# ishine/Prior-DiffuSE

Measured on AMD Instinct MI355X. Metric: enhanced-audio sec/sec (RTF), 6-step fast sampling, B=32, higher is better.
Workload: dtype f16x2; 1 GPU; B=32 x 4 s 16 kHz utterances per GPU, [B,2,401,161] spectrograms, GCRN prior + DiffUNet1 6-step sampling, STFT..ISTFT, seeded random weights; global_batch=32, frames=401, parallelism=batch-shard x1, graph=True, streams_per_gpu=1, batches_in_flight=3

## Files before the change

prior-diffuse_amd/csrc/gconv4.hip:

```cpp
#include <hip/hip_runtime.h>
#include <stdint.h>
#include <stdio.h>
#include <stdlib.h>

#include "pdse.h"
#include "pdse_internal.h"

#include "gconv_common.h"

#ifndef G4_CH
#define G4_CH 3
#endif

__device__ __forceinline__ float g4_load(const float* sbase, const unsigned byte_off) {
  float v;
  asm volatile("global_load_dword %0, %1, %2" : "=v"(v) : "v"(byte_off), "s"(sbase) : "memory");
  return v;
}
typedef float g4_f32x4 __attribute__((ext_vector_type(4)));
__device__ __forceinline__ g4_f32x4 g4_load16(const float* sbase, const unsigned byte_off) {
  g4_f32x4 v;
  asm volatile("global_load_dwordx4 %0, %1, %2" : "=v"(v) : "v"(byte_off), "s"(sbase) : "memory");
  return v;
}
// ... 308 lines not shown
    const int tap = kb / cbn, cb = kb - tap * cbn;
    int dt = 0, df = 0;
#pragma unroll
    for (int k = 0; k < 12; ++k) {
      dt = tap == k ? d.tap_dt[k] : dt;
      df = tap == k ? d.tap_df[k] : df;
    }
    const int tin = t + dt, fin = df;
    const bool inb = pvalid && fin >= 0 && fin < d.Fin && tin >= 0 && tin < d.Tin;
    const int64_t pos = inb ? (int64_t)b * d.in0.sb + (int64_t)tin * d.in0.st + (int64_t)fin * d.in0.sf : 0;
    float x[8];
    if constexpr (BLK) {
      const float* q = d.in0.ptr + pos + (int64_t)(2 * cb + h) * d.in0.sc;
      const float4 v0 = *reinterpret_cast<const float4*>(q), v1 = *reinterpret_cast<const float4*>(q + 4);
      x[0] = v0.x, x[1] = v0.y, x[2] = v0.z, x[3] = v0.w, x[4] = v1.x, x[5] = v1.y, x[6] = v1.z, x[7] = v1.w;
    } else {
      const float* q = d.in0.ptr + pos + (int64_t)(16 * cb + 8 * h) * d.in0.sc;
#pragma unroll
      for (int e = 0; e < 8; ++e) x[e] = q[(int64_t)e * d.in0.sc];
    }
#pragma unroll
    for (int e = 0; e < 8; ++e) x[e] = inb ? x[e] : 0.f;
    if (elu) {
#pragma unroll
      for (int e = 0; e < 8; ++e) x[e] = x[e] < 0.f ? fast_exp(x[e]) - 1.0f : x[e];
    }
    uint4 bp[NP];
    split_planes<NP>(x, bp, pow2i(PDSE_F16_ACT_EXP));
#pragma unroll
    for (int p = 0; p < NP; ++p) bimg[(kb * NP + p) * 64 + lane] = bp[p];
  }
  __syncthreads();

  const int mt0 = (blockIdx.y * 8 + wave) * MTW;
  if (mt0 >= mtiles) return;
  const uint4* const wl = reinterpret_cast<const uint4*>(d.w0) + lane;
  u32x4 a[MTW][NP];
  auto lda = [&](const int kb, const int m) {
    const u32x4* src = reinterpret_cast<const u32x4*>(wl + ((size_t)kb * mtiles + mt0 + m) * (NP * 64));
#pragma unroll
    for (int p = 0; p < NP; ++p) a[m][p] = src[p * 64];
  };
  f32x16 acc[MTW];
#pragma unroll
  for (int m = 0; m < MTW; ++m) {
#pragma unroll
    for (int r = 0; r < 16; ++r) acc[m][r] = 0.f;
    lda(0, m);
  }
  for (int kb = 0; kb < nkb; ++kb) {
    uint4 bp[NP];
#pragma unroll
    for (int p = 0; p < NP; ++p) bp[p] = bimg[(kb * NP + p) * 64 + lane];
    const int kn = min(kb + 1, nkb - 1);
#pragma unroll
    for (int m = 0; m < MTW; ++m) {
      acc[m] = g4_mma<NP>(a[m], bp, acc[m]);
      lda(kn, m);
    }
  }
  if constexpr (NP == 2) {
    const float us = pow2i(-(PDSE_F16_ACT_EXP + d.wexp));
#pragma unroll
    for (int m = 0; m < MTW; ++m)
#pragma unroll
      for (int r = 0; r < 16; ++r) acc[m][r] *= us;
  }
  gconv_epilogue_impl<PDSE_EPI_LINEAR, MTW, true>(d, tail_from_desc(d), acc, acc, b, t, 0, pvalid, lane, h, mt0, mtiles, 0);
}

template <bool BLK, int NP>
static int launch4f(const pdse_gconv_desc* d, hipStream_t s) {
  constexpr int MTW = 4;
  const int mtiles = (d->Cout + 31) / 32, nkb = d->ntaps * (d->in0.C >> 4);
  const long long N = (long long)d->B * d->Tout;
  const dim3 grid((unsigned)((N + 31) / 32), (mtiles + 8 * MTW - 1) / (8 * MTW)), block(512);
  const size_t lds = (size_t)nkb * NP * 64 * sizeof(uint4);
  static unsigned long long attr_mask = 0;
  if (lds > 64 * 1024 && pdse_lds_attr((const void*)gconv4_flat_kernel<MTW, BLK, NP>, &attr_mask, "gconv4 flat lds attribute")) return 1;
  hipLaunchKernelGGL((gconv4_flat_kernel<MTW, BLK, NP>), grid, block, lds, s, *d);
  return pdse_check_launch("gconv4 flat");
}

static int check4(const pdse_gconv_desc* d) {
  const bool two = d->in1.C > 0;
  const long long span0 = 4 * ((long long)d->B * d->in0.sb + 40ll * d->in0.sc), span1 = two ? 4 * ((long long)d->B * d->in1.sb + 40ll * d->in1.sc) : 0;
  auto blk_ok = [](const pdse_src& x) {
    return x.blk == 0 || (x.blk == 8 && !((x.sb | x.sc | x.st | x.sf) & 3) && (reinterpret_cast<uintptr_t>(x.ptr) & 15) == 0);
  };
  if (!blk_ok(d->in0) || (two && !blk_ok(d->in1)) || (two && d->in0.blk != d->in1.blk)) {
    pdse_set_error("gconv4: a channel-blocked source has blk = 8, strides in multiples of 4 floats and a 16-byte aligned base; "
                   "two sources are both blocked or both plain");
    return 1;
  }
  if (!(d->epi == PDSE_EPI_LINEAR || d->epi == PDSE_EPI_GLU) || (d->in0.C & 15) || (d->in1.C & 15) || d->in0.C == 0 || d->cin1 ||
      d->xf_mode != 0 || d->padrow != nullptr || d->ntaps > 12 || span0 >= (1ll << 32) || span1 >= (1ll << 32) ||
      (d->epi == PDSE_EPI_GLU && !d->w1) || (d->korder == 5 && (d->wexp < -40 || d->wexp > 40))) {
    pdse_set_error("gconv4: split-bf16 GEMM convolutions need LINEAR / GLU, channel counts in multiples of 16, <= 12 taps, "
                   "no load transform / pad row, 32-bit gather offsets");
    return 1;
  }
  if (d->flat && (d->flat != 1 || !(d->korder == 3 || d->korder == 5) || d->epi != PDSE_EPI_LINEAR || two || d->Fout != 1 ||
                  d->ntaps * (d->in0.C >> 4) > 32 || (d->Cout & 255) || d->out_cr != 1 || (long long)d->B * d->Tout > (1ll << 30))) {
    pdse_set_error("gconv4: the flat form takes korder 3 / 5 LINEAR launches of one source with Fout = 1, ntaps * C <= 512, "
                   "Cout in multiples of 256 and out_cr = 1");
    return 1;
  }
  return 0;
}

int pdse_gconv4_launch(const pdse_gconv_desc* d, hipStream_t s) {
  if (check4(d)) return 1;
  if (d->flat) {
    if (d->korder == 5) return d->in0.blk ? launch4f<true, 2>(d, s) : launch4f<false, 2>(d, s);
    return d->in0.blk ? launch4f<true, 3>(d, s) : launch4f<false, 3>(d, s);
  }
  const int mtiles = (d->Cout + 31) / 32;
  if (d->epi == PDSE_EPI_GLU) return mtiles >= 2 ? launch4<PDSE_EPI_GLU, 2>(d, s, mtiles) : launch4<PDSE_EPI_GLU, 1>(d, s, mtiles);
  if (mtiles >= 4) return launch4<PDSE_EPI_LINEAR, 4>(d, s, mtiles);
  if (mtiles >= 2) return launch4<PDSE_EPI_LINEAR, 2>(d, s, mtiles);
  return launch4<PDSE_EPI_LINEAR, 1>(d, s, mtiles);
}

template <int MT, bool BLK>
__global__ __launch_bounds__(512, 2) void gconv4_pair_kernel(const pdse_gconv_desc d, const pdse_gconv_desc e) {
  constexpr int NP = 2, FB = 64 * NP;
  constexpr int FR = 2 * MT, FR2 = 2 * FR;
  extern __shared__ uint4 ring[];
  const unsigned ring_base = (unsigned)(uintptr_t)ring;
  const int tid = threadIdx.x;
  const int lane = tid & 63, wave = tid >> 6;
  const int col = lane & 31, h = lane >> 5;
  const int b = blockIdx.y;
  const int P = d.Tout * d.Fout;
  const int p = (blockIdx.x * 8 + wave) * 32 + col;
  const bool pvalid = p < P;
  const int t = pvalid ? p / d.Fout : 0;
  const int j = pvalid ? p - t * d.Fout : 0;
  const int mtiles = (d.Cout + 31) >> 5;
  const int mt0 = blockIdx.z * MT;

  const int cbn0 = d.in0.C >> 4, cbn1 = d.in1.C >> 4;
  const int cps0 = (cbn0 + G4_CH - 1) / G4_CH, cps1 = (cbn1 + G4_CH - 1) / G4_CH;
  const int nch0 = d.ntaps * cps0, nch = nch0 + d.ntaps * cps1;

  auto uni = [](const int v) { return __builtin_amdgcn_readfirstlane(v); };
  auto decode = [&](const int ci) {
    g4_chunk c;
    c.s = uni(ci >= nch0);
    const int q = c.s ? ci - nch0 : ci, cps = c.s ? cps1 : cps0, cbn = c.s ? cbn1 : cbn0;
    c.tap = uni(q / cps);
    c.cb0 = uni((q - c.tap * cps) * G4_CH);
    c.n = uni(min(G4_CH, cbn - c.cb0));
    c.kb0 = uni((c.s ? d.ntaps * cbn0 : 0) + c.tap * cbn + c.cb0);
    return c;
  };
  auto dma = [&](const g4_chunk& c, const int buf) {
    const int nf = c.tap == 0 ? FR2 : FR;
    const int kb1 = (c.s ? cbn0 : 0) + c.cb0;
    const int npieces = c.n * nf * NP;
    for (int pc = __builtin_amdgcn_readfirstlane(wave); pc < npieces; pc += 8) {
      const int i = pc / (nf * NP), rem = pc - i * (nf * NP), f = rem / NP, part = rem - f * NP;
      const bool odd = f >= FR;
      const int g = odd ? f - FR : f, br = g / MT, m = g - br * MT;
      if (mt0 + m < mtiles) {
        const float* const w = odd ? (br ? e.w1 : e.w0) : (br ? d.w1 : d.w0);
        const uint4* src = reinterpret_cast<const uint4*>(w) + ((size_t)((odd ? kb1 : c.kb0) + i) * mtiles + mt0 + m) * FB + part * 64 + lane;
        glds16(src, ring + ((buf * G4_CH + i) * FR2 + f) * FB + part * 64);
      }
    }
  };
  auto gather = [&](const g4_chunk& c, g4_raw<BLK>& raw, bool& inb) {
    const bool s1 = c.s != 0;
    const float* const sptr = s1 ? d.in1.ptr : d.in0.ptr;
    const int64_t ssb = s1 ? d.in1.sb : d.in0.sb, ssc = s1 ? d.in1.sc : d.in0.sc, sst = s1 ? d.in1.st : d.in0.st,
                  ssf = s1 ? d.in1.sf : d.in0.sf;
    int dt = 0, df = 0;
#pragma unroll
    for (int k = 0; k < 12; ++k) {
      dt = c.tap == k ? d.tap_dt[k] : dt;
      df = c.tap == k ? d.tap_df[k] : df;
    }
    const int tin = t + dt, fin = j * d.sf_in + df;
    inb = pvalid && fin >= 0 && fin < d.Fin && tin >= 0 && tin < d.Tin;
    if constexpr (BLK) {
      const unsigned off = 4u * (unsigned)((inb ? (int64_t)b * ssb + (int64_t)tin * sst + (int64_t)fin * ssf : 0) + (int64_t)h * ssc);
#pragma unroll
      for (int i = 0; i < G4_CH; ++i) {
        if (i < c.n) {
          const float* base = sptr + (int64_t)(2 * (c.cb0 + i)) * ssc;
          raw.v[i][0] = g4_load16(base, off);
          raw.v[i][1] = g4_load16(base + 4, off);
        }
      }
    } else {
// ... 135 lines not shown
```

prior-diffuse_amd/nets.py:

```python
import ctypes as C

import numpy as np
import torch

from . import _lib as L
from . import packing as P

F0 = 161
BIG = 1 << 30

TAG_NONE, TAG_EPS_BLOCK, TAG_EPS_CONV1, TAG_TCM, TAG_PRIOR, TAG_LSTM, TAG_SIGNAL, TAG_EW = range(8)


class WeightBank:

    def __init__(self):
        self.items = {}
        self.keep = []
        self.owners = []

    def token(self, obj):
        if obj is None:
            return None
        for i, o in enumerate(self.owners):
# ... 132 lines not shown
            if hit is None:
                raise RuntimeError("range audit: the f16x2 operand at 0x%x lies in no buffer the builder named (PlanBase.named)" % addr)
            name, t = hit
            key = (name + suffix, kind)
            if key in seen:
                continue
            seen.add(key)
            out.append((name + suffix, t, kind, P.F16_ACT_EXP if kind == L.RANGE_F32 else 0,
                        None if box is None else dict(box, off=(addr - t.data_ptr()) // 2)))
        return out

    def finish(self):
        if self.plan is not None:
            self.plan.keep(self.ctx.keep, self.ctx.bank)

    def src(self, t, C_, sb, sc, st, sf, off=0, act=L.ACT_NONE, blk=0):
        return L.Src(Ctx.ptr(t, off), sb, sc, st, sf, C_, act, blk, 0)

    def gconv(self, *, in0, in1=None, Tin, Fin, taps, sf_in, W, Cout, bias0=None, bias0_sb=0,
              bias1=None, bias1_sb=0, epi=L.EPI_LINEAR, act=L.ACT_NONE, act_slope=0.0,
              padrow=None, padrow_sb=0, padrow_off=0, cin1=False, resid=None, out,
              out_strides, out_off=0, out_cr=1, B, Tout, Fout, tag=TAG_NONE, bias0_off=0, phase1=None, nx=None,
              bias1_off=0, bias_t0=None, label="gconv", s3=False, s3g=False, has_xf=False, flat=False):
        ctx = self.ctx
        d = L.GconvDesc()
        d.in0 = in0
        d.in1 = in1 if in1 is not None else L.Src(0, 0, 0, 0, 0, 0, 0)
        d.Tin, d.Fin = Tin, Fin
        d.padrow, d.padrow_sb = Ctx.ptr(padrow, padrow_off), padrow_sb
        ttaps = tuple((int(a), int(b)) for a, b in taps)
        tkey = ("taps", ttaps)
        tp = ctx.bank.items.get(tkey)
        if tp is None:
            ctx._banking += 1
            tp = ctx.bank.items[tkey] = self._up(P.taps_array(ttaps))
            ctx._banking -= 1
        d.taps, d.ntaps, d.sf_in = tp.data_ptr(), len(ttaps), sf_in
        for i, (dt_, df_) in enumerate(ttaps[:12]):
            d.tap_dt[i], d.tap_df[i] = dt_, df_
        d.cin1 = 1 if cin1 else 0
        c0, c1 = d.in0.C, d.in1.C
        pipelined_ok = padrow is None and not self.force_generic
        s3 = bool(s3) and pipelined_ok and epi == L.EPI_BIGLU and (
            ((c0, c1) == (32, 0) and len(ttaps) in (4, 6)) or ((c0, c1, len(ttaps)) == (2, 2, 10) and phase1 is None))
        s3g = (bool(s3g) and not s3 and pipelined_ok and epi in (L.EPI_LINEAR, L.EPI_GLU) and not cin1 and not has_xf
               and c0 > 0 and c0 % 16 == 0 and c1 % 16 == 0 and len(ttaps) <= 12)
        site = "%s:%d:%d:%d:%d:%d:%d:%d:%d" % (label, epi, len(ttaps), c0, c1, Cout, pipelined_ok, s3, s3g)
        if s3g:
            pack = lambda: P.gconv_gemm_fields(W(), len(ttaps), c0, c1, self.gemm_planes)
        elif s3:
            pack = lambda: P.gconv_s3_fields(W(), len(ttaps), c0 + c1)
        else:
            pack = lambda: P.gconv_fields(W(), len(ttaps), c0, c1, epi, cin1, pipelined_ok)
        self.apply(d, self.fields(site, pack))
        d.Cout = Cout
        if bias0 is not None:
            d.bias0 = Ctx.ptr(bias0, bias0_off)
        if bias1 is not None:
            d.bias1 = Ctx.ptr(bias1, bias1_off)
        d.bias0_sb, d.bias1_sb = bias0_sb, bias1_sb
        if bias_t0 is not None:
            d.bias0_t0, d.bias1_t0 = Ctx.ptr(bias_t0[0], bias_t0[1]), Ctx.ptr(bias_t0[0], bias_t0[2])
        d.epi, d.act, d.act_slope = epi, act, float(act_slope)
        if phase1 is not None and d.korder in (1, 2):
            d.p1mask, d.Fout1 = phase1["mask"], phase1["Fout1"]
        elif phase1 is not None and d.korder == 5 and epi == L.EPI_GLU:
            d.p1mask, d.Fout1 = phase1["mask"], phase1["Fout1"]
        if nx is not None:
            tiles = nx["tiles"]
            d.nx_n, d.nx_keep, d.nx_row0 = len(tiles), 1 if nx.get("keep") else 0, nx.get("row0", -1)
            for i, tl in enumerate(tiles):
                if tl.get("bias") is not None:
                    d.nx_bias[i] = Ctx.ptr(tl["bias"], tl.get("bias_off", 0))
                d.nx_bias_sb[i] = tl.get("bias_sb", 0)
                d.nx_out[i] = Ctx.ptr(tl["out"])
                d.nx_sb[i], d.nx_sc[i], d.nx_st[i], d.nx_sf[i] = tl["strides"]
                d.nx_off[i] = tl.get("off", 0)
                d.nx_add[i] = Ctx.ptr(tl.get("add"))
        d.resid = Ctx.ptr(resid)
        d.out = Ctx.ptr(out)
        d.out_sb, d.out_sc_hi, d.out_sc_lo, d.out_st, d.out_sf = out_strides
        d.out_off, d.out_cr = out_off, out_cr
        d.B, d.Tout, d.Fout = B, Tout, Fout
        d.flat = 1 if flat and s3g and d.korder in (3, 5) else 0
        self.add(d, tag)
        return d


def nchw(C_, T, F):
    return C_ * T * F, T * F, F, 1


def nchw_out(C_, T, F):
    return C_ * T * F, T * F, 0, F, 1


def nc8(C_, T, F):
    return C_ * T * F, T * F * 8, F * 8, 8


def nc8_out(C_, T, F):
    return C_ * T * F, T * F * 8, 1, F * 8, 8


class EpsNetPlan(PlanBase):

    ENC_F = [161, 79, 39, 19, 9, 4]
    fused_tcm = True
    chain_conv1 = True
    compose_stage1 = True
    split_bf16 = True
    split_tcm = True
    plane_h = True
    tcm_stack = True
    parity_planes = True
    planes = 2
    TCM_F16 = True
    NSLOT = 20

    def __init__(self, ctx, sd, B, T, time_cond=True, nsteps=1, plan=None, table=None, with_pre=None, split_bf16=None,
                 planes=None, plane_h=None, exclusive=False, frames=None):
        with_pre = time_cond if with_pre is None else with_pre
        if split_bf16 is not None:
            self.split_bf16 = bool(split_bf16)
        if planes is not None:
            if int(planes) not in (1, 2, 3):
                raise ValueError("planes is 3 (bf16x3), 2 (f16x2) or 1 (bf16 mode)")
            self.planes = int(planes)
        if plane_h is not None:
            self.plane_h = bool(plane_h)
        if self.planes == 1:
            self.plane_h = True
        self.tcm_planes = 3 if (self.planes == 2 and not self.TCM_F16) else self.planes
        self.use_tcm_stack = bool(self.tcm_stack and exclusive)
        self.frames = frames
        if frames is not None and (self.force_generic or not self.fused_tcm):
            raise ValueError("exact ragged batches need a fused TCM form (csrc/tcm.hip, csrc/tcm2.hip): the three-launch form has no frames table")
        self.sd = sd
        ok = (self.split_bf16 and self.chain_conv1 and self.compose_stage1 and time_cond and with_pre and not self.force_generic
              and all(float(P._np(sd[k])[0]) <= 1.0 for k in sd if k.endswith(".weight") and P._np(sd[k]).shape == (1,)))
        if not ok:
            if self.planes == 1:
                raise ValueError("bf16 mode needs the chained split-bf16 DiffUNet1 path (PReLU slopes <= 1)")
            self.plane_h = False
            if self.planes == 2:
                self.planes = self.tcm_planes = 3
        super().__init__(ctx, plan, ns=(ctx.bank.token(sd), bool(time_cond), bool(with_pre), self.fused_tcm, self.chain_conv1,
                                        self.compose_stage1, self.split_bf16, self.split_tcm,
                                        ctx.bank.token(table), str(self.plane_h), self.planes, self.parity_planes))
        self.sd, self.B, self.T, self.time_cond, self.nsteps = sd, B, T, time_cond, nsteps
        self.with_pre = with_pre
        a = ctx.alloc
        self.x = a(B, 2, T, F0)
        self.x_init = a(B, 2, T, F0) if self.with_pre else None
        self.out = a(B, 2, T, F0)
        self.H = a(B, 32, T + 1, F0)
        self.H2 = a(B, 32, T + 1, F0)
        self.Pskip = [[None] + [a(B + 1, 32, T, self.ENC_F[k]) for k in range(1, 5)] for _ in range(2)]
        self.zero32 = self.upw("zero32", lambda: np.zeros(32))
        self.en = [a(B, 64, T, f) for f in self.ENC_F[1:5]] + [a(B, 64, 4, T)]
        self.tcm_a, self.tcm_b = a(B, 256, T), a(B, 256, T)
        self.tcm_h, self.tcm_g = a(B, 64, T), a(B, 64, T)
        self.tcm_hs = [ctx.alloc_u16(*P.tcm2_hs_shape(B, T, self.tcm_planes)) for _ in range(2)]
        self._tcm_stack = None
        self.tcm_flags = torch.zeros(B * ((T + 31) // 32), dtype=torch.int32, device=ctx.device)
        self.tcm_status = torch.zeros(4, dtype=torch.int32, device=ctx.device)
        ctx.keep += [self.tcm_flags, self.tcm_status]
# ... 502 lines not shown
            if chained and k == 1 and self.compose_stage1:
                Fin = self._biconvglu_composed(step, src_x, src_i, o, ostr, nx)
            else:
                Fin = self._biconvglu(step, k, src_x, src_i, Fin, o, ostr, H=Hc, do_conv1=(k == 1 or not chained), nx=nx)
            if chained:
                Hc, Hn = Hn, Hc
            src_x, src_i = self.src(o, 64, *nchw(64, T, Fin)), None
        cur, nxt = self.en[4], self.tcm_a
        names = [("TCMs.%d.residual%d" % (i, j + 1), dil) for i in range(3) for j, dil in enumerate((1, 2, 4, 8, 16, 32))]
        if self.force_generic or not self.fused_tcm:
            for p, dil in names:
                self._residual(p, dil, cur, nxt)
                cur, nxt = nxt, (self.tcm_b if nxt is self.tcm_a else self.tcm_a)
        elif self.split_bf16 and self.split_tcm:
            hcur, hnxt = self.tcm_hs
            self._residual_split(None, 1, cur, None, None, hcur, names[0][0], mode=1)
            self._tcm_stack = [] if self.use_tcm_stack else None
            for n, (p, dil) in enumerate(names):
                p_next = names[n + 1][0] if n + 1 < len(names) else None
                self._residual_split(p, dil, cur, nxt, hcur, hnxt, p_next)
                cur, nxt = nxt, (self.tcm_b if nxt is self.tcm_a else self.tcm_a)
                hcur, hnxt = hnxt, hcur
            if self._tcm_stack:
                sd_ = L.Tcm2sDesc()
                for n, blk in enumerate(self._tcm_stack):
                    sd_.blk[n] = blk
                sd_.n = len(self._tcm_stack)
                sd_.flags, sd_.status = self.tcm_flags.data_ptr(), self.tcm_status.data_ptr()
                self.add(sd_, TAG_TCM)
            self._tcm_stack = None
        else:
            hcur, hnxt = self.tcm_h, self.tcm_g
            self._tcm_conv1(names[0][0], cur, hcur)
            for n, (p, dil) in enumerate(names):
                p_next = names[n + 1][0] if n + 1 < len(names) else None
                self._residual_fused(p, dil, cur, nxt, hcur, hnxt, p_next)
                cur, nxt = nxt, (self.tcm_b if nxt is self.tcm_a else self.tcm_a)
                hcur, hnxt = hnxt, hcur
        tcm_out = cur
        if self._plane_stage("dec"):
            self._decoders_planes(step, tcm_out, out)
            return out
        for di, de in enumerate(("de_real", "de_imag")):
            in0 = self.src(tcm_out, 64, 256 * T, 4 * T, 1, T)
            Fin = 4
            Hc, Hn = self.H, self.H2
            for n, k in enumerate((5, 4, 3, 2, 1)):
                skip = self.en[k - 1]
                if k == 5:
                    in1 = self.src(skip, 64, 256 * T, 4 * T, 1, T)
                else:
                    in1 = self.src(skip, 64, *nchw(64, T, self.ENC_F[k]))
                p = "%s.de%d.0" % (de, k)
                if k > 1:
                    o, ooff = self.dec[n & 1], 0
                    fn = lambda Fo: nchw_out(64, T, Fo)
                    bn, pr = "%s.de%d.2" % (de, k), "%s.de%d.3.weight" % (de, k)
                else:
                    o, ooff = out, di * T * F0
                    fn = lambda Fo: nchw_out(2, T, Fo)
                    bn, pr = None, None
                nx = None
                if chained and k > 1:
                    Fo = 2 * (Fin - 1) + 3
                    wn = lambda de=de, k=k: self.w("%s.de%d.0.conv1.weight" % (de, k - 1))[:, :, 0, 0].T[:, :64]
                    nx = dict(keep=False, row0=-1, tiles=[dict(wfn=wn, bias=self.zero32, out=Hn, add=self.Pskip[di][k - 1],
                                                                strides=(32 * T * Fo, T * Fo, Fo, 2))])
                Fin = self._biconvtransglu(step, 5 + 5 * di + n, p, k, in0, in1, Fin, o, fn, bn, pr, out_off=ooff, H=Hc,
                                           do_conv1=(k == 5 or not chained), nx=nx)
                if chained:
                    Hc, Hn = Hn, Hc
                in0 = self.src(o, 64, *nchw(64, T, Fin))
        return out


class GcrnPlan(PlanBase):
    fused_last = True
    fused_glstm = True
    split_bf16 = True
    gemm_planes = 2
    block8 = True
    fuse_phases = True
    flat_proj = True
    persist_lstm = True
    chunk_proj = True
    CHUNK_TC = 32
    PERSIST_MAX_B = 4
    ENC_C = [2, 16, 32, 64, 128, 256]
    ENC_F = [161, 80, 39, 19, 9, 4]

    def __init__(self, ctx, sd, B, T, plan=None, split_bf16=None, exclusive=False, planes=None):
        if split_bf16 is not None:
            self.split_bf16 = bool(split_bf16)
        if planes is not None:
            if planes not in (1, 2, 3) or (planes in (1, 2) and not self.split_bf16):
                raise ValueError("planes is 3 (bf16x3), 2 (f16x2) or 1 (bf16 mode); the one- and two-plane forms run on the GEMM kernels (split_bf16)")
            self.gemm_planes = int(planes)
        self.persist = bool(self.persist_lstm and self.fused_glstm and exclusive and B <= self.PERSIST_MAX_B and not self.force_generic)
        self.exclusive = bool(exclusive)
        self.chunk = bool(self.chunk_proj and self.fused_glstm and not exclusive and not self.persist and not self.force_generic
                          and T >= 2 * self.CHUNK_TC)
        super().__init__(ctx, plan, ns=(ctx.bank.token(sd), self.fused_last, self.fused_glstm, self.split_bf16, self.block8, self.persist,
                                        self.gemm_planes))
        self.sd, self.B, self.T = sd, B, T
        a = ctx.alloc
        self.Bp = Bp = (B + 31) // 32 * 32
        self.status = None
        self.x = a(B, 2, T, F0)
        self.out = a(B, 2, T, F0)
        self.e = [a(B, self.ENC_C[i + 1], T, self.ENC_F[i + 1]) for i in range(5)]
        self.gx = a(2, T, 2048, Bp, zero=True)
        R = 2 * self.CHUNK_TC if self.chunk else 2
        self.hT = a(R, 2, 512, Bp, zero=True)
        self.cst = a(2, 512, Bp, zero=True)
        self.y = a(B, T, 1024)
        if self.persist:
            bq = 1 << (B - 1).bit_length()
            self.gran = torch.zeros(4 * 1024 * bq, dtype=torch.int64, device=ctx.device)
            self.status = torch.zeros(4, dtype=torch.int32, device=ctx.device)
            ctx.keep += [self.gran, self.status]
        elif self.fused_glstm and not self.force_generic:
            self.hT2, self.cst2 = a(2, 2, 512, Bp, zero=True), a(2, 512, Bp, zero=True)
            self.gx2, self.part = a(R, 2, 2048, Bp, zero=True), a(R, 2, 64, Bp, 2, zero=True)
        else:
            self.yn = a(B, 1024, T)
        self.glstm = a(B, 256, T, 4)
        self.d = [a(B, 128, T, 9), a(B, 64, T, 19), a(B, 32, T, 39), a(B, 16, T, 80), a(B, 1, T, 161)]
        for i, t_ in enumerate(self.e):
            self.named("gcrn.e%d" % (i + 1), t_)
        self.named("gcrn.glstm", self.glstm)
        for i, t_ in enumerate(self.d[:4]):
            self.named("gcrn.d%d" % (5 - i), t_)
        self.named("gcrn.x", self.x)

    def w(self, k):
        return P._np(self.sd[k])

    def _nchw(self, t, blocked):
        if blocked and self.split_bf16 and not self.force_generic and self.block8:
            B, C_, T, F = t.shape
            return t.view(B, C_ // 8, T, F, 8).permute(0, 1, 4, 2, 3).reshape(B, C_, T, F)
        return t

    def enc_out(self, k):
        return self._nchw(self.e[k - 1], k >= 2)

    def glstm_out(self):
        return self._nchw(self.glstm, True)

    def _lstm_proj(self, layer, proj, gx_lay):
        B, T, Bp = self.B, self.T, self.Bp
        for g in range(2):
            p = "glstm.%s.%d." % (layer, g)
            in0, Tin, Fin, taps, wk_fn, Tout, Fout, ost, osf = proj(g)
            self.gconv(in0=in0, Tin=Tin, Fin=Fin, taps=taps, sf_in=1, Cout=2048,
                       W=lambda p=p, wk_fn=wk_fn: dict(wk0=wk_fn(self.w(p + "weight_ih_l0")),
                                                       bias0=self.w(p + "bias_ih_l0") + self.w(p + "bias_hh_l0")),
                       out=self.gx, out_strides=gx_lay + (0, ost, osf), out_off=g * T * 2048 * Bp, B=B, Tout=Tout, Fout=Fout,
                       tag=TAG_PRIOR, label=p + "ih", s3g=self.split_bf16,
                       flat=self.flat_proj and Fout == 1 and len(taps) * in0.C <= 512)

    def _lstm_layer(self, layer, xproj_src_fn, y_su, y_sg):
        B, T, Bp = self.B, self.T, self.Bp
        self._lstm_proj(layer, xproj_src_fn, (1, Bp))

        def pack_whh():
            return P.pack_lstm_whh([self.w("glstm.%s.%d.weight_hh_l0" % (layer, g)) for g in range(2)])

        d = L.LstmDesc()
        d.gx, d.whh = self.gx.data_ptr(), self.upw(layer + ".whh", pack_whh).data_ptr()
        d.hT, d.cst, d.y = self.hT.data_ptr(), self.cst.data_ptr(), self.y.data_ptr()
        d.y_sb, d.y_st, d.y_su, d.y_sg = T * 1024, 1024, y_su, y_sg
        d.B, d.Bp, d.T, d.H, d.G = B, Bp, T, 512, 2
        self.add(d, TAG_LSTM)

    def _glstm_natural(self):
        per = lambda key: [self.w("glstm.%s" % (key % g)) for g in range(2)]
        return (per("lstm_list1.%d.weight_hh_l0"), per("lstm_list2.%d.weight_ih_l0"), per("lstm_list2.%d.bias_ih_l0"),
                per("lstm_list2.%d.bias_hh_l0"), per("lstm_list2.%d.weight_hh_l0"), self.w("glstm.ln1.weight"), self.w("glstm.ln1.bias"))

    def _glstm_wavefront(self, proj1):
        B, T, Bp = self.B, self.T, self.Bp
        self._lstm_proj("lstm_list1", proj1, (2048, 1))
        d = L.GlstmDesc()
        self.apply(d, self.fields("glstm.wavefront", lambda: P.pack_glstm_wavefront(*self._glstm_natural())))
        d.gx1, d.gx2, d.part = self.gx.data_ptr(), self.gx2.data_ptr(), self.part.data_ptr()
        d.hT1, d.cst1, d.hT2, d.cst2 = self.hT.data_ptr(), self.cst.data_ptr(), self.hT2.data_ptr(), self.cst2.data_ptr()
        d.y, d.y_sb, d.y_st, d.y_su, d.y_sg = self.y.data_ptr(), T * 1024, 1024, 1, 512
        d.B, d.Bp, d.T, d.H, d.G, d.eps = B, Bp, T, 512, 2, 1e-5
        d.slices = 2 if self.exclusive else 1
        if self.chunk:
            d.tc, d.lag = self.CHUNK_TC, self.CHUNK_TC + 1
        self.add(d, TAG_LSTM)

    def _glstm_persistent(self, proj1):
        B, T, Bp = self.B, self.T, self.Bp
        self._lstm_proj("lstm_list1", proj1, (2048, 1))
        d = L.GlstmpDesc()
        self.apply(d, self.fields("glstm.persistent", lambda: P.pack_glstm_persistent(*self._glstm_natural())))
        d.gx1, d.gran, d.status = self.gx.data_ptr(), self.gran.data_ptr(), self.status.data_ptr()
        d.y, d.y_sb, d.y_st, d.y_su, d.y_sg = self.y.data_ptr(), T * 1024, 1024, 1, 512
        d.B, d.Bp, d.T, d.H, d.G, d.eps = B, Bp, T, 512, 2, 1e-5
        self.add(d, TAG_LSTM)

    def _ln(self, name, out_t, osb, os_hi, os_lo, os_t, r, blk=0):
        d = L.LnDesc()
        d.blk = blk
        d.in_, d.out = self.y.data_ptr(), out_t.data_ptr()
        d.gamma = self.upw(name + ".g", lambda: self.w(name + ".weight")).data_ptr()
        d.beta = self.upw(name + ".b", lambda: self.w(name + ".bias")).data_ptr()
        d.osb, d.os_hi, d.os_lo, d.os_t = osb, os_hi, os_lo, os_t
        d.B, d.T, d.N, d.r, d.eps = self.B, self.T, 1024, r, 1e-5
        self.add(d, TAG_PRIOR)

    def build(self, x=None, out=None):
        B, T, Bp = self.B, self.T, self.Bp
        x = self.x if x is None else x
        out = self.out if out is None else out
        blk = self.split_bf16 and not self.force_generic and self.block8

        def lay(k_is_blocked, C_, Fq):
            if k_is_blocked:
                return nc8(C_, T, Fq), nc8_out(C_, T, Fq), 8
            return nchw(C_, T, Fq), nchw_out(C_, T, Fq), 1

        src = self.src(x, 2, *nchw(2, T, F0))
        e_lay = [lay(blk and k >= 2, self.ENC_C[k], self.ENC_F[k]) for k in range(1, 6)]
        for k in range(1, 6):
            ci, co, Fin, Fout = self.ENC_C[k - 1], self.ENC_C[k], self.ENC_F[k - 1], self.ENC_F[k]
            kk, taps = P.conv_taps(1, 3, 0)
            p = "conv%d" % k
            ist, ost_, ocr = e_lay[k - 1]
            self.gconv(in0=src, Tin=T, Fin=Fin, taps=taps, sf_in=2, Cout=co, epi=L.EPI_GLU, act=L.ACT_ELU,
                       W=lambda p=p, k=k, kk=kk: dict(wk0=P.conv_kmat(self.sd[p + ".conv1.weight"], kk),
                                                      wk1=P.conv_kmat(self.sd[p + ".conv2.weight"], kk),
                                                      bias0=self.w(p + ".conv1.bias"), bias1=self.w(p + ".conv2.bias"),
                                                      post=P.bn_fold(self.sd, "bn%d" % k)),
                       out=self.e[k - 1], out_strides=ost_, out_cr=ocr, B=B, Tout=T, Fout=Fout, tag=TAG_PRIOR, label=p,
                       s3g=self.split_bf16)
            src = self.src(self.e[k - 1], co, *ist, blk=8 if ocr == 8 else 0)

        def proj1(g):
            wk = lambda Wih: np.concatenate([Wih[:, f::4].T for f in range(4)], axis=0)
            s = self.src(self.e[4], 128, *e_lay[4][0], off=128 * g * T * 4, blk=8 if blk else 0)
            return s, T, 4, [(0, f) for f in range(4)], wk, T, 1, 2048 * Bp, 0

        if self.persist:
            self._glstm_persistent(proj1)
        elif self.fused_glstm and not self.force_generic:
            self._glstm_wavefront(proj1)
        else:
            self._lstm_layer("lstm_list1", proj1, y_su=2, y_sg=1)
            self._ln("glstm.ln1", self.yn, 1024 * T, T, 0, 1, 1)

            def proj2(g):
                s = self.src(self.yn, 512, 1024 * T, T, 0, 1, off=512 * g * T)
                return s, 1, T, [(0, 0)], (lambda Wih: Wih.T), 1, T, 0, 2048 * Bp

            self._lstm_layer("lstm_list2", proj2, y_su=1, y_sg=512)
        if blk:
            self._ln("glstm.ln2", self.glstm, 256 * T * 4, T * 4 * 8, 8, 4 * 8, 4, blk=8)
        else:
            self._ln("glstm.ln2", self.glstm, 256 * T * 4, T * 4, 1, 4, 4)

        dec = [(5, 512, 128), (4, 256, 64), (3, 128, 32), (2, 64, 16), (1, 32, 1)]
        for br in (1, 2):
            in0 = self.src(self.glstm, 256, *(nc8(256, T, 4) if blk else nchw(256, T, 4)), blk=8 if blk else 0)
            in1 = self.src(self.e[4], 256, *e_lay[4][0], blk=8 if blk else 0)
            Fin = 4
            for n, (k, ci, co) in enumerate(dec):
                p = "conv%d_t_%d" % (k, br)
                Fout = 2 * (Fin - 1) + 3 + (1 if k == 2 else 0)
                if k == 1 and self.fused_last and not self.force_generic:
                    g = L.GcrnLastDesc()
                    self.apply(g, self.fields(p + ".last", lambda p=p, br=br: P.gcrn_last_fields(self.sd, p, br)))
                    g.in0, g.in1 = self.d[3].data_ptr(), self.e[0].data_ptr()
                    g.out, g.out_sb = Ctx.ptr(out, (br - 1) * T * F0), 2 * T * F0
                    g.B, g.T = B, T
                    self.add(g, TAG_PRIOR)
                    break
                dblk = blk and k >= 3
                fuse = self.fuse_phases and self.split_bf16 and self.gemm_planes == 2 and not self.force_generic
                ist, (osb, osc, olo, ost, osf), ocr = lay(dblk, co, Fout)
                for phase in (0, 1):
                    kk, taps = P.convT_phase_taps(1, 3, phase)
                    self.gconv(in0=in0, in1=in1, Tin=T, Fin=Fin, taps=taps, sf_in=1, Cout=co, epi=L.EPI_GLU, act=L.ACT_ELU,
                               W=lambda p=p, k=k, br=br, kk=kk: dict(
                                   wk0=P.convT_kmat(self.sd[p + ".conv1.weight"], kk),
                                   wk1=P.convT_kmat(self.sd[p + ".conv2.weight"], kk), bias0=self.w(p + ".conv1.bias"),
                                   bias1=self.w(p + ".conv2.bias"), post=P.bn_fold(self.sd, "bn%d_t_%d" % (k, br))),
                               out=self.d[n], out_strides=(osb, osc, olo, ost, 2 * osf), out_off=phase * osf, out_cr=ocr, B=B,
                               Tout=T, Fout=(Fout - phase + 1) // 2, tag=TAG_PRIOR, label="%s.ph%d" % (p, phase),
                               s3g=self.split_bf16, phase1=dict(mask=1, Fout1=Fout // 2) if phase == 0 and fuse and co <= 32 else None)
                Fin = Fout
                if k > 1:
                    in0 = self.src(self.d[n], co, *ist, blk=8 if dblk else 0)
                    skip = self.e[k - 2]
                    sblk = e_lay[k - 2][2] == 8
                    in1 = self.src(skip, co, *e_lay[k - 2][0], act=L.ACT_ELU, blk=8 if sblk else 0)
            else:
                self.gconv(in0=self.src(self.d[4], 1, *nchw(1, T, F0)), Tin=T, Fin=F0, taps=[(0, f) for f in range(F0)],
                           sf_in=1, W=lambda br=br: dict(wk0=self.w("fc%d.weight" % br).T, bias0=self.w("fc%d.bias" % br)),
                           Cout=F0, cin1=True, out=out, out_strides=(2 * T * F0, 1, 0, F0, 0), out_off=(br - 1) * T * F0, B=B,
                           Tout=T, Fout=1, tag=TAG_PRIOR, label="fc%d" % br)
        return out


def feat_ns(feat_type):
    return () if feat_type == "sqrt" else (feat_type,)


class StftPlan(PlanBase):

    def __init__(self, ctx, B, L_, plan=None, normalize=True, split_bf16=False, reflect_own=False, feat_type="sqrt"):
        self.feat_type = L.feat_type_of(feat_type)
        super().__init__(ctx, plan, ns=("stft", bool(split_bf16)) + feat_ns(feat_type))
        self.split_bf16 = bool(split_bf16)
        if L_ <= 160:
            raise ValueError(f"utterance of {L_} samples: the centred STFT reflects 160 samples on each side (torch.stft "
                             "raises for the same input)")
        self.B, self.L = B, L_
        self.T = 1 + L_ // 160
        self.wav = ctx.alloc(B, L_)
        self.xpad = ctx.alloc(B, L_ + 320)
        self.c = ctx.alloc(B)
        self.lens = torch.full((B,), L_, dtype=torch.int32, device=ctx.device)
        ctx.keep.append(self.lens)
        self.feat = ctx.alloc(B, 2, self.T, F0)
        self.normalize = normalize
        self.reflect_own = bool(reflect_own)

    def build(self, feat=None, prep=True):
        B, L_, T = self.B, self.L, self.T
        feat = self.feat if feat is None else feat
        if prep:
            d = L.WavprepDesc()
            d.wav, d.xpad, d.c, d.lens = self.wav.data_ptr(), self.xpad.data_ptr(), self.c.data_ptr(), self.lens.data_ptr()
            d.B, d.L, d.pad, d.normalize = B, L_, 160, 1 if self.normalize else 0
            d.reflect_own = 1 if self.reflect_own else 0
            self.add(d, TAG_SIGNAL)
        Lp = L_ + 320
        self.gconv(in0=self.src(self.xpad, 320, Lp, 1, 0, 1), Tin=1, Fin=Lp, taps=[(0, 0)],
                   sf_in=160, W=lambda: dict(wk0=P.stft_kmat(320)), Cout=2 * F0, out=feat, label="stft",
                   out_strides=(2 * T * F0, T * F0, 1, 0, F0), out_cr=F0, B=B, Tout=1, Fout=T, tag=TAG_SIGNAL,
                   s3g=self.split_bf16)
        mode = L.COMPRESS_MODE[self.feat_type]
        if mode is not None:
            c = L.CompandDesc()
            c.in_, c.out, c.plane, c.B, c.mode = feat.data_ptr(), feat.data_ptr(), T * F0, B, mode
            self.add(c, TAG_SIGNAL)
        return feat


class IstftPlan(PlanBase):

    def __init__(self, ctx, B, T, L_, plan=None, split_bf16=False, frames=None, lens=None, feat_type="sqrt"):
        self.feat_type = L.feat_type_of(feat_type)
        super().__init__(ctx, plan, ns=("istft", bool(split_bf16)) + feat_ns(feat_type))
        self.frames_tab, self.lens_tab = frames, lens
        self.split_bf16 = bool(split_bf16)
        self.B, self.T, self.L = B, T, L_
        self.spec = ctx.alloc(B, 2, T, F0)
        self.dec = ctx.alloc(B, T, 2 * P.ISTFT_ROW, zero=True)
        self.frames = ctx.alloc(B, 320, T)
        self.wav = ctx.alloc(B, L_)
        self.win2 = self.upw("win2", lambda: P.hann_periodic(320) ** 2)

    def build(self, spec=None, c=None):
        B, T = self.B, self.T
        spec = self.spec if spec is None else spec
        cd = L.CompandDesc()
        cd.in_, cd.out, cd.plane, cd.B, cd.mode = spec.data_ptr(), self.dec.data_ptr(), T * F0, B, L.DECOMPRESS_MODE[self.feat_type]
        K = 2 * P.ISTFT_ROW
        cd.out_sb, cd.out_sc, cd.out_st, cd.F = T * K, P.ISTFT_ROW, K, F0
        self.add(cd, TAG_SIGNAL)
        self.gconv(in0=self.src(self.dec, K, T * K, 1, K, 0), Tin=T, Fin=1, taps=[(0, 0)],
# ... 392 lines not shown
```

Measured before the change: 10040 audio_s/s.

## Add shared-gather GLU conv kernel for deep GCRN encoder/decoder stages

Adds a new gconv4 kernel variant in which all waves of a block cooperatively gather and split input activations into LDS once, in chunks of 8 K-blocks, and each wave then reuses that staged B operand across its own 32-channel output tile and two position tiles. It is enabled for conv4, conv5 and conv5_t.ph0 of the GCRN prior, where many output channels share a small spatial extent. The goal is to stop each output-channel tile from gathering the same activations redundantly. In exchange it adds block-wide barriers per chunk and a serialized epilogue, and it only handles 64, 128 or 256 output channels.

```diff
diff --git a/prior-diffuse_amd/csrc/gconv4.hip b/prior-diffuse_amd/csrc/gconv4.hip
--- a/prior-diffuse_amd/csrc/gconv4.hip
+++ b/prior-diffuse_amd/csrc/gconv4.hip
@@ -414,6 +414,146 @@
   return pdse_check_launch("gconv4 flat");
 }
 
+#define G4S_PT 2
+#define G4S_KB 8
+template <int NW, bool BLK, int NP>
+__global__ __launch_bounds__(64 * NW, 3) void gconv4_shared_kernel(const pdse_gconv_desc d) {
+  extern __shared__ uint4 bimg[];
+  const int tid = threadIdx.x;
+  const int lane = tid & 63, wave = __builtin_amdgcn_readfirstlane(tid >> 6);
+  const int col = lane & 31, h = lane >> 5;
+  const int b = blockIdx.y;
+  const int P = d.Tout * d.Fout;
+  bool pvalid[G4S_PT];
+  int t[G4S_PT], j[G4S_PT];
+#pragma unroll
+  for (int q = 0; q < G4S_PT; ++q) {
+    const int p = (blockIdx.x * G4S_PT + q) * 32 + col;
+    pvalid[q] = p < P;
+    t[q] = pvalid[q] ? p / d.Fout : 0;
+    j[q] = pvalid[q] ? p - t[q] * d.Fout : 0;
+  }
+  const int mtiles = NW;
+  const int cbn0 = d.in0.C >> 4, cbn1 = d.in1.C >> 4;
+  const int nkb0 = d.ntaps * cbn0, nkb = nkb0 + d.ntaps * cbn1;
+
+  auto stage = [&](const int kb, const int i) {
+    const bool s1 = kb >= nkb0;
+    const int r = s1 ? kb - nkb0 : kb, cbn = s1 ? cbn1 : cbn0;
+    const int tap = r / cbn, cb = r - tap * cbn;
+    const float* const sptr = s1 ? d.in1.ptr : d.in0.ptr;
+    const int64_t ssb = s1 ? d.in1.sb : d.in0.sb, ssc = s1 ? d.in1.sc : d.in0.sc, sst = s1 ? d.in1.st : d.in0.st,
+                  ssf = s1 ? d.in1.sf : d.in0.sf;
+    const bool elu = (s1 ? d.in1.act : d.in0.act) == PDSE_ACT_ELU;
+    int dt = 0, df = 0;
+#pragma unroll
+    for (int k = 0; k < 12; ++k) {
+      dt = tap == k ? d.tap_dt[k] : dt;
+      df = tap == k ? d.tap_df[k] : df;
+    }
+#pragma unroll
+    for (int q = 0; q < G4S_PT; ++q) {
+    const int tin = t[q] + dt, fin = j[q] * d.sf_in + df;
+    const bool inb = pvalid[q] && fin >= 0 && fin < d.Fin && tin >= 0 && tin < d.Tin;
+    const int64_t pos = inb ? (int64_t)b * ssb + (int64_t)tin * sst + (int64_t)fin * ssf : 0;
+    float x[8];
+    if constexpr (BLK) {
+      const float* g = sptr + pos + (int64_t)(2 * cb + h) * ssc;
+      const float4 v0 = *reinterpret_cast<const float4*>(g), v1 = *reinterpret_cast<const float4*>(g + 4);
+      x[0] = v0.x, x[1] = v0.y, x[2] = v0.z, x[3] = v0.w, x[4] = v1.x, x[5] = v1.y, x[6] = v1.z, x[7] = v1.w;
+    } else {
+      const float* g = sptr + pos + (int64_t)(16 * cb + 8 * h) * ssc;
+#pragma unroll
+      for (int e = 0; e < 8; ++e) x[e] = g[(int64_t)e * ssc];
+    }
+#pragma unroll
+    for (int e = 0; e < 8; ++e) x[e] = inb ? x[e] : 0.f;
+    if (elu) {
+#pragma unroll
+      for (int e = 0; e < 8; ++e) x[e] = x[e] < 0.f ? fast_exp(x[e]) - 1.0f : x[e];
+    }
+    uint4 bp[NP];
+    split_planes<NP>(x, bp, pow2i(PDSE_F16_ACT_EXP));
+#pragma unroll
+    for (int p = 0; p < NP; ++p) bimg[((i * G4S_PT + q) * NP + p) * 64 + lane] = bp[p];
+    }
+  };
+
+  const uint4* const wl0 = reinterpret_cast<const uint4*>(d.w0) + lane;
+  const uint4* const wl1 = reinterpret_cast<const uint4*>(d.w1) + lane;
+  u32x4 a[2][NP];
+  auto lda = [&](const int kb) {
+    const size_t o = ((size_t)kb * mtiles + wave) * (NP * 64);
+    const u32x4* s0 = reinterpret_cast<const u32x4*>(wl0 + o);
+    const u32x4* s1 = reinterpret_cast<const u32x4*>(wl1 + o);
+#pragma unroll
+    for (int p = 0; p < NP; ++p) a[0][p] = s0[p * 64], a[1][p] = s1[p * 64];
+  };
+  f32x16 acc0[G4S_PT], acc1[G4S_PT];
+#pragma unroll
+  for (int q = 0; q < G4S_PT; ++q)
+#pragma unroll
+    for (int r = 0; r < 16; ++r) acc0[q][r] = acc1[q][r] = 0.f;
+  lda(0);
+  for (int kb0 = 0; kb0 < nkb; kb0 += G4S_KB) {
+    const int n = min(G4S_KB, nkb - kb0);
+    if (kb0) __syncthreads();
+#pragma unroll 1
+    for (int i = wave; i < n; i += NW) stage(kb0 + i, i);
+    __syncthreads();
+#pragma unroll 1
+    for (int i = 0; i < n; ++i) {
+      uint4 bp[G4S_PT][NP];
+#pragma unroll
+      for (int q = 0; q < G4S_PT; ++q)
+#pragma unroll
+        for (int p = 0; p < NP; ++p) bp[q][p] = bimg[((i * G4S_PT + q) * NP + p) * 64 + lane];
+#pragma unroll
+      for (int q = 0; q < G4S_PT; ++q) {
+        acc0[q] = g4_mma<NP>(a[0], bp[q], acc0[q]);
+        acc1[q] = g4_mma<NP>(a[1], bp[q], acc1[q]);
+      }
+      lda(min(kb0 + i + 1, nkb - 1));
+    }
+  }
+  if constexpr (NP == 2) {
+    const float us = pow2i(-(PDSE_F16_ACT_EXP + d.wexp));
+#pragma unroll
+    for (int q = 0; q < G4S_PT; ++q)
+#pragma unroll
+      for (int r = 0; r < 16; ++r) acc0[q][r] *= us, acc1[q][r] *= us;
+  }
+  static_assert(G4S_PT == 2, "the epilogue loop selects between two position tiles");
+  const pdse_tail tl = tail_from_desc(d);
+  __builtin_assume(wave >= 0 && wave < NW);
+  pdse_gconv_desc dd = d;
+  dd.Cout = 32 * NW;
+#pragma unroll 1
+  for (int q = 0; q < G4S_PT; ++q) {
+    f32x16 m = q ? acc0[1] : acc0[0], g = q ? acc1[1] : acc1[0];
+    int lq = lane;
+    asm volatile("" : "+v"(lq));
+    gconv_epilogue<PDSE_EPI_GLU, 1>(dd, tl, &m, &g, b, q ? t[1] : t[0], q ? j[1] : j[0], q ? pvalid[1] : pvalid[0], lq, lq >> 5, wave, mtiles);
+  }
+}
+
+template <int NW, bool BLK, int NP>
+static int launch4s(const pdse_gconv_desc* d, hipStream_t s) {
+  const int P = d->Tout * d->Fout;
+  const dim3 grid(((P + 31) / 32 + G4S_PT - 1) / G4S_PT, d->B), block(64 * NW);
+  const size_t lds = (size_t)G4S_KB * G4S_PT * NP * 64 * sizeof(uint4);
+  static unsigned long long attr_mask = 0;
+  if (lds > 64 * 1024 && pdse_lds_attr((const void*)gconv4_shared_kernel<NW, BLK, NP>, &attr_mask, "gconv4 shared lds attribute")) return 1;
+  hipLaunchKernelGGL((gconv4_shared_kernel<NW, BLK, NP>), grid, block, lds, s, *d);
+  return pdse_check_launch("gconv4 shared");
+}
+
+template <int NW>
+static int launch4s(const pdse_gconv_desc* d, hipStream_t s) {
+  if (d->korder == 5) return d->in0.blk ? launch4s<NW, true, 2>(d, s) : launch4s<NW, false, 2>(d, s);
+  return d->in0.blk ? launch4s<NW, true, 3>(d, s) : launch4s<NW, false, 3>(d, s);
+}
+
 static int check4(const pdse_gconv_desc* d) {
   const bool two = d->in1.C > 0;
   const long long span0 = 4 * ((long long)d->B * d->in0.sb + 40ll * d->in0.sc), span1 = two ? 4 * ((long long)d->B * d->in1.sb + 40ll * d->in1.sc) : 0;
@@ -432,6 +572,14 @@
                    "no load transform / pad row, 32-bit gather offsets");
     return 1;
   }
+  if (d->flat == 2) {
+    if (!(d->korder == 3 || d->korder == 5) || d->epi != PDSE_EPI_GLU || !(d->Cout == 64 || d->Cout == 128 || d->Cout == 256) ||
+        (long long)d->Tout * d->Fout > (1ll << 30)) {
+      pdse_set_error("gconv4: flat form 2 (shared gather) takes korder 3 / 5 GLU launches of 64, 128 or 256 output channels");
+      return 1;
+    }
+    return 0;
+  }
   if (d->flat && (d->flat != 1 || !(d->korder == 3 || d->korder == 5) || d->epi != PDSE_EPI_LINEAR || two || d->Fout != 1 ||
                   d->ntaps * (d->in0.C >> 4) > 32 || (d->Cout & 255) || d->out_cr != 1 || (long long)d->B * d->Tout > (1ll << 30))) {
     pdse_set_error("gconv4: the flat form takes korder 3 / 5 LINEAR launches of one source with Fout = 1, ntaps * C <= 512, "
@@ -443,6 +591,7 @@
 
 int pdse_gconv4_launch(const pdse_gconv_desc* d, hipStream_t s) {
   if (check4(d)) return 1;
+  if (d->flat == 2) return d->Cout == 256 ? launch4s<8>(d, s) : d->Cout == 128 ? launch4s<4>(d, s) : launch4s<2>(d, s);
   if (d->flat) {
     if (d->korder == 5) return d->in0.blk ? launch4f<true, 2>(d, s) : launch4f<false, 2>(d, s);
     return d->in0.blk ? launch4f<true, 3>(d, s) : launch4f<false, 3>(d, s);
diff --git a/prior-diffuse_amd/nets.py b/prior-diffuse_amd/nets.py
--- a/prior-diffuse_amd/nets.py
+++ b/prior-diffuse_amd/nets.py
@@ -238,7 +238,7 @@
         d.out_sb, d.out_sc_hi, d.out_sc_lo, d.out_st, d.out_sf = out_strides
         d.out_off, d.out_cr = out_off, out_cr
         d.B, d.Tout, d.Fout = B, Tout, Fout
-        d.flat = 1 if flat and s3g and d.korder in (3, 5) else 0
+        d.flat = int(flat) if flat and s3g and d.korder in (3, 5) else 0
         self.add(d, tag)
         return d
 
@@ -907,6 +907,8 @@
     block8 = True
     fuse_phases = True
     flat_proj = True
+    shared_gather = True
+    SHARED_STAGES = frozenset(("conv4", "conv5", "conv5_t.ph0"))
     persist_lstm = True
     chunk_proj = True
     CHUNK_TC = 32
@@ -1062,7 +1064,7 @@
                                                       bias0=self.w(p + ".conv1.bias"), bias1=self.w(p + ".conv2.bias"),
                                                       post=P.bn_fold(self.sd, "bn%d" % k)),
                        out=self.e[k - 1], out_strides=ost_, out_cr=ocr, B=B, Tout=T, Fout=Fout, tag=TAG_PRIOR, label=p,
-                       s3g=self.split_bf16)
+                       s3g=self.split_bf16, flat=2 if self.shared_gather and p in self.SHARED_STAGES else 0)
             src = self.src(self.e[k - 1], co, *ist, blk=8 if ocr == 8 else 0)
 
         def proj1(g):
@@ -1116,7 +1118,8 @@
                                    bias1=self.w(p + ".conv2.bias"), post=P.bn_fold(self.sd, "bn%d_t_%d" % (k, br))),
                                out=self.d[n], out_strides=(osb, osc, olo, ost, 2 * osf), out_off=phase * osf, out_cr=ocr, B=B,
                                Tout=T, Fout=(Fout - phase + 1) // 2, tag=TAG_PRIOR, label="%s.ph%d" % (p, phase),
-                               s3g=self.split_bf16, phase1=dict(mask=1, Fout1=Fout // 2) if phase == 0 and fuse and co <= 32 else None)
+                               s3g=self.split_bf16, phase1=dict(mask=1, Fout1=Fout // 2) if phase == 0 and fuse and co <= 32 else None,
+                               flat=2 if self.shared_gather and "conv%d_t.ph%d" % (k, phase) in self.SHARED_STAGES else 0)
                 Fin = Fout
                 if k > 1:
                     in0 = self.src(self.d[n], co, *ist, blk=8 if dblk else 0)
```

Result: no change. 10090 audio_s/s, median of 6 (+0.5%).
